# coreperf/rejit

Measured on AMD Instinct MI355X. Metric: GB/s text scanned (regexdna 9 patterns, 50M-line input); matches/s alongside, higher is better.
Workload: dtype u8

## Files before the change

### rejit_amd/csrc/plane_count.hip

```cpp
#include <hip/hip_runtime.h>
#include <hip/hip_ext.h>

#include <cstdlib>

#include "exact_count.h"
#include "kernels.h"
#include "plane_codes.h"
#include "short_walk.h"
#include "stream_load.h"
#include "wave_ops.h"

namespace rejit_amd {

namespace {

constexpr uint64_t kBlock = 2048;
constexpr uint32_t kPieceB = 1024;
constexpr uint32_t kStashWords = (2048 + 16) / 4;
#ifndef RJ_PC_RING
#define RJ_PC_RING 256
#endif
constexpr uint32_t kRing = RJ_PC_RING;

__device__ __forceinline__ uint32_t codes16(const uint4& v, const PlaneCodes& k) {
  const uint32_t s = k.shift;
  return (codes4(v.x, k) >> s) | (codes4(v.y, k) << (8 - s)) | (codes4(v.z, k) << (16 - s)) | (codes4(v.w, k) << (24 - s));
}

struct Raw {
  uint4 a, b;
};

__device__ __forceinline__ void load_block(const uint8_t* block, uint32_t lane_off, Raw& r) {
  r.a = stream_load16(block + lane_off);
  r.b = stream_load16(block + lane_off + kPieceB);
}

__device__ __forceinline__ uint32_t guarded_dword(const uint8_t* text, uint64_t n, uint64_t at) {
  uint32_t v = 0;
#pragma unroll
  for (int k = 0; k < 4; k++)
    if (at + k < n) v |= static_cast<uint32_t>(text[at + k]) << (8 * k);
  return v;
}

template <int NB>
__device__ __forceinline__ uint32_t plane_test(uint32_t ta, uint32_t tb, uint32_t ha, uint32_t hb, const PlaneCountParams& a) {
  constexpr uint32_t kEven = 0x55555555u;
  const uint32_t L = (ta & kEven) | ((tb << 1) & ~kEven);
  const uint32_t H = ((ta >> 1) & kEven) | (tb & ~kEven);
  const uint32_t Ln = (ha & kEven) | ((hb << 1) & ~kEven);
  const uint32_t Hn = ((ha >> 1) & kEven) | (hb & ~kEven);
  register uint32_t q0 asm("v48") = ~(L | H);
  register uint32_t q1 asm("v49") = L & ~H;
  register uint32_t q2 asm("v50") = ~L & H;
  register uint32_t q3 asm("v51") = L & H;
  register uint32_t n0 asm("v52") = ~(Ln | Hn);
  register uint32_t n1 asm("v53") = Ln & ~Hn;
  register uint32_t n2 asm("v54") = ~Ln & Hn;
  register uint32_t n3 asm("v55") = Ln & Hn;
  uint32_t codes = ~a.mask_bits;
  asm volatile("" : "+s"(codes));
  auto code = [&](int b, int i) { return (codes >> (16 * b + 2 * i)) & 3u; };
  uint32_t E[8][NB], Z[NB], O[NB];
#pragma unroll
  for (int half = 0; half < 2; half++) {
    if (NB == 1) {
      if (half == 0) {
      asm volatile(
          "s_set_gpr_idx_on %[c00], 0x3\n"
          "v_mov_b32 %[e00], v48\n"
          "s_set_gpr_idx_idx %[c10]\n"
          "v_alignbit_b32 %[e10], v52, v48, 2\n"
          "s_set_gpr_idx_idx %[c20]\n"
          "v_alignbit_b32 %[e20], v52, v48, 4\n"
          "s_set_gpr_idx_idx %[c30]\n"
          "v_alignbit_b32 %[e30], v52, v48, 6\n"
          "s_set_gpr_idx_off\n"
          : [e00] "=&v"(E[0][0]), [e10] "=&v"(E[1][0]), [e20] "=&v"(E[2][0]), [e30] "=&v"(E[3][0])
          : [c00] "s"(code(0, 0)), [c10] "s"(code(0, 1)), [c20] "s"(code(0, 2)), [c30] "s"(code(0, 3)), "v"(q0), "v"(q1), "v"(q2), "v"(q3), "v"(n0), "v"(n1), "v"(n2), "v"(n3));
      } else {
      asm volatile(
          "s_set_gpr_idx_on %[c40], 0x3\n"
          "v_alignbit_b32 %[e40], v52, v48, 8\n"
          "s_set_gpr_idx_idx %[c50]\n"
          "v_alignbit_b32 %[e50], v52, v48, 10\n"
          "s_set_gpr_idx_idx %[c60]\n"
          "v_alignbit_b32 %[e60], v52, v48, 12\n"
          "s_set_gpr_idx_idx %[c70]\n"
          "v_alignbit_b32 %[e70], v52, v48, 14\n"
          "s_set_gpr_idx_off\n"
          : [e40] "=&v"(E[4][0]), [e50] "=&v"(E[5][0]), [e60] "=&v"(E[6][0]), [e70] "=&v"(E[7][0])
          : [c40] "s"(code(0, 4)), [c50] "s"(code(0, 5)), [c60] "s"(code(0, 6)), [c70] "s"(code(0, 7)), "v"(q0), "v"(q1), "v"(q2), "v"(q3), "v"(n0), "v"(n1), "v"(n2), "v"(n3));
      }
    } else {
      if (half == 0) {
      asm volatile(
          "s_set_gpr_idx_on %[c00], 0x3\n"
          "v_mov_b32 %[e00], v48\n"
          "s_set_gpr_idx_idx %[c01]\n"
          "v_mov_b32 %[e01], v48\n"
          "s_set_gpr_idx_idx %[c10]\n"
          "v_alignbit_b32 %[e10], v52, v48, 2\n"
          "s_set_gpr_idx_idx %[c11]\n"
          "v_alignbit_b32 %[e11], v52, v48, 2\n"
          "s_set_gpr_idx_idx %[c20]\n"
          "v_alignbit_b32 %[e20], v52, v48, 4\n"
          "s_set_gpr_idx_idx %[c21]\n"
          "v_alignbit_b32 %[e21], v52, v48, 4\n"
          "s_set_gpr_idx_idx %[c30]\n"
          "v_alignbit_b32 %[e30], v52, v48, 6\n"
          "s_set_gpr_idx_idx %[c31]\n"
          "v_alignbit_b32 %[e31], v52, v48, 6\n"
          "s_set_gpr_idx_off\n"
          : [e00] "=&v"(E[0][0]), [e01] "=&v"(E[0][1]), [e10] "=&v"(E[1][0]), [e11] "=&v"(E[1][1]), [e20] "=&v"(E[2][0]), [e21] "=&v"(E[2][1]), [e30] "=&v"(E[3][0]), [e31] "=&v"(E[3][1])
          : [c00] "s"(code(0, 0)), [c01] "s"(code(1, 0)), [c10] "s"(code(0, 1)), [c11] "s"(code(1, 1)), [c20] "s"(code(0, 2)), [c21] "s"(code(1, 2)), [c30] "s"(code(0, 3)), [c31] "s"(code(1, 3)), "v"(q0), "v"(q1), "v"(q2), "v"(q3), "v"(n0), "v"(n1), "v"(n2), "v"(n3));
      } else {
      asm volatile(
          "s_set_gpr_idx_on %[c40], 0x3\n"
          "v_alignbit_b32 %[e40], v52, v48, 8\n"
          "s_set_gpr_idx_idx %[c41]\n"
          "v_alignbit_b32 %[e41], v52, v48, 8\n"
          "s_set_gpr_idx_idx %[c50]\n"
          "v_alignbit_b32 %[e50], v52, v48, 10\n"
          "s_set_gpr_idx_idx %[c51]\n"
          "v_alignbit_b32 %[e51], v52, v48, 10\n"
          "s_set_gpr_idx_idx %[c60]\n"
          "v_alignbit_b32 %[e60], v52, v48, 12\n"
          "s_set_gpr_idx_idx %[c61]\n"
          "v_alignbit_b32 %[e61], v52, v48, 12\n"
          "s_set_gpr_idx_idx %[c70]\n"
          "v_alignbit_b32 %[e70], v52, v48, 14\n"
          "s_set_gpr_idx_idx %[c71]\n"
          "v_alignbit_b32 %[e71], v52, v48, 14\n"
          "s_set_gpr_idx_off\n"
          : [e40] "=&v"(E[4][0]), [e41] "=&v"(E[4][1]), [e50] "=&v"(E[5][0]), [e51] "=&v"(E[5][1]), [e60] "=&v"(E[6][0]), [e61] "=&v"(E[6][1]), [e70] "=&v"(E[7][0]), [e71] "=&v"(E[7][1])
          : [c40] "s"(code(0, 4)), [c41] "s"(code(1, 4)), [c50] "s"(code(0, 5)), [c51] "s"(code(1, 5)), [c60] "s"(code(0, 6)), [c61] "s"(code(1, 6)), [c70] "s"(code(0, 7)), [c71] "s"(code(1, 7)), "v"(q0), "v"(q1), "v"(q2), "v"(q3), "v"(n0), "v"(n1), "v"(n2), "v"(n3));
      }
    }
#pragma unroll
    for (int i = 4 * half; i < 4 * half + 4; i++)
#pragma unroll
      for (int b = 0; b < NB; b++) {
        const uint32_t e = E[i][b];
        if (i == 0) {
          Z[b] = e;
        } else if (i == 1) {
          O[b] = Z[b] | e;
          Z[b] &= e;
        } else {
          O[b] = Z[b] | (O[b] & e);
          if (i < 7) Z[b] &= e;
        }
      }
  }
  return NB > 1 ? (O[0] | O[NB - 1]) : O[0];
}


struct Lens {
  uint64_t w[2];
};
static_assert(kMaxFused <= 24, "two words of twelve lengths");
__device__ __forceinline__ uint32_t len_of(const Lens& l, uint32_t p) {
  return static_cast<uint32_t>((p < 12 ? l.w[0] >> (5 * p) : l.w[1] >> (5 * (p - 12))) & 31u);
}

}

template <int NB>
struct ExactShape {
  using Args = PlaneCountParams;
  static constexpr uint32_t kFixedLen = 8;
  static constexpr bool kBlobInLds = false;
  static constexpr bool kList = false;
  static constexpr bool kCapture = true;
  __device__ static __forceinline__ const PlaneCountParams& common(const Args& g) { return g; }
  __device__ static __forceinline__ uint32_t lmax(const Args&) { return 8u; }
  __device__ static __forceinline__ uint32_t offset_of(const Args&, const uint32_t*, uint32_t) { return 0u; }
  __device__ static __forceinline__ uint32_t test(uint32_t ta, uint32_t tb, uint32_t ha, uint32_t hb, const Args& g) { return plane_test<NB>(ta, tb, ha, hb, g); }
  __device__ static __forceinline__ void classify(const Args& a, const uint32_t* table, uint64_t pos, bool have, uint32_t& mask, Lens&) {
    const bool ok = have && pos >= a.sb && pos < a.se && pos + 8 <= a.n;
    uint32_t lo = 0, hi = 0;
    if (ok) {
      __builtin_memcpy(&lo, a.text + pos, 4);
      __builtin_memcpy(&hi, a.text + pos + 4, 4);
    }
    mask = exact_classify<NB>(table, a.base_lo, a.base_hi, lo, hi);
    mask = ok ? mask : 0u;
  }
  __device__ static __forceinline__ void classify_bytes(const Args& a, const uint32_t* table, uint64_t pos, bool have, uint32_t lo, uint32_t hi, uint32_t& mask) {
    const bool ok = have && pos >= a.sb && pos < a.se && pos + 8 <= a.n;
    mask = exact_classify<NB>(table, a.base_lo, a.base_hi, lo, hi);
    mask = ok ? mask : 0u;
  }
};

template <int NB>
struct ListShape {
  using Args = PlaneListParams;
  static constexpr uint32_t kFixedLen = 8;
  static constexpr bool kBlobInLds = false;
  static constexpr bool kList = true;
  static constexpr bool kCapture = false;
  __device__ static __forceinline__ void classify_bytes(const Args&, const uint32_t*, uint64_t, bool, uint32_t, uint32_t, uint32_t& mask) { mask = 0; }
  __device__ static __forceinline__ const PlaneCountParams& common(const Args& g) { return g.c; }
  __device__ static __forceinline__ uint32_t lmax(const Args&) { return 8u; }
  __device__ static __forceinline__ uint32_t offset_of(const Args&, const uint32_t*, uint32_t) { return 0u; }
  __device__ static __forceinline__ uint32_t test(uint32_t ta, uint32_t tb, uint32_t ha, uint32_t hb, const Args& g) { return plane_test<NB>(ta, tb, ha, hb, g.c); }
  __device__ static __forceinline__ void classify(const Args&, const uint32_t*, uint64_t, bool, uint32_t& mask, Lens&) { mask = 0; }
};

namespace {

template <bool TOL>
__device__ __forceinline__ uint32_t general_test(uint32_t ta, uint32_t tb, uint32_t ha, uint32_t hb, const PlaneCountGParams& g) {
  constexpr uint32_t kEven = 0x55555555u;
  const uint32_t L = (ta & kEven) | ((tb << 1) & ~kEven);
  const uint32_t H = ((ta >> 1) & kEven) | (tb & ~kEven);
  const uint32_t Ln = (ha & kEven) | ((hb << 1) & ~kEven);
  const uint32_t Hn = ((ha >> 1) & kEven) | (hb & ~kEven);
  register uint32_t q0 asm("v48") = ~(L | H);
  register uint32_t q1 asm("v49") = L & ~H;
  register uint32_t q2 asm("v50") = ~L & H;
  register uint32_t q3 asm("v51") = L & H;
  register uint32_t q4 asm("v52") = ~0u;
  register uint32_t n0 asm("v56") = ~(Ln | Hn);
  register uint32_t n1 asm("v57") = Ln & ~Hn;
  register uint32_t n2 asm("v58") = ~Ln & Hn;
  register uint32_t n3 asm("v59") = Ln & Hn;
  register uint32_t n4 asm("v60") = ~0u;
  uint32_t c = 0;
#pragma clang loop unroll(disable)
  for (uint32_t b = 0; b < g.c.n_bases; b++) {
    const uint32_t* ix = g.idx[b];
    uint32_t e0, e1, e2, e3, e4, e5, e6, e7;
    asm volatile(
        "s_set_gpr_idx_on %[i0], 0x3\n"
        "v_mov_b32 %[e0], v48\n"
        "s_set_gpr_idx_idx %[i1]\n"
        "v_alignbit_b32 %[e1], v56, v48, 2\n"
        "s_set_gpr_idx_idx %[i2]\n"
        "v_alignbit_b32 %[e2], v56, v48, 4\n"
        "s_set_gpr_idx_idx %[i3]\n"
        "v_alignbit_b32 %[e3], v56, v48, 6\n"
        "s_set_gpr_idx_idx %[i4]\n"
        "v_alignbit_b32 %[e4], v56, v48, 8\n"
        "s_set_gpr_idx_idx %[i5]\n"
        "v_alignbit_b32 %[e5], v56, v48, 10\n"
        "s_set_gpr_idx_idx %[i6]\n"
        "v_alignbit_b32 %[e6], v56, v48, 12\n"
        "s_set_gpr_idx_idx %[i7]\n"
        "v_alignbit_b32 %[e7], v56, v48, 14\n"
        "s_set_gpr_idx_off\n"
        : [e0] "=&v"(e0), [e1] "=&v"(e1), [e2] "=&v"(e2), [e3] "=&v"(e3), [e4] "=&v"(e4), [e5] "=&v"(e5), [e6] "=&v"(e6), [e7] "=&v"(e7)
        : [i0] "s"(ix[0]), [i1] "s"(ix[1]), [i2] "s"(ix[2]), [i3] "s"(ix[3]), [i4] "s"(ix[4]), [i5] "s"(ix[5]), [i6] "s"(ix[6]), [i7] "s"(ix[7]), "v"(q0), "v"(q1), "v"(q2),
          "v"(q3), "v"(q4), "v"(n0), "v"(n1), "v"(n2), "v"(n3), "v"(n4));
    if (TOL) {
      uint32_t Z = e0, O = e0 | e1;
      Z &= e1;
      O = Z | (O & e2);
      Z &= e2;
      O = Z | (O & e3);
      Z &= e3;
      O = Z | (O & e4);
      Z &= e4;
      O = Z | (O & e5);
      Z &= e5;
      O = Z | (O & e6);
      Z &= e6;
      O = Z | (O & e7);
      c |= O;
    } else {
      const uint32_t z0 = e0 & e1 & e2, z1 = e3 & e4 & e5;
      c |= z0 & z1 & e6 & e7;
    }
  }
  return c;
}

}

template <int W, int MAXK, bool TOL>
struct GeneralShape {
  using Args = PlaneCountGParams;
  static constexpr uint32_t kFixedLen = 0;
  static constexpr bool kBlobInLds = true;
  static constexpr bool kList = false;
  static constexpr bool kCapture = false;
  __device__ static __forceinline__ void classify_bytes(const Args&, const uint32_t*, uint64_t, bool, uint32_t, uint32_t, uint32_t& mask) { mask = 0; }
  __device__ static __forceinline__ const PlaneCountParams& common(const Args& g) { return g.c; }
  __device__ static __forceinline__ uint32_t lmax(const Args& g) { return g.lmax; }
  __device__ static __forceinline__ uint32_t offset_of(const Args&, const uint32_t* blob, uint32_t p) {
    return reinterpret_cast<const ClassifyDesc*>(blob)[p].win_offset;
  }
  __device__ static __forceinline__ uint32_t test(uint32_t ta, uint32_t tb, uint32_t ha, uint32_t hb, const Args& g) { return general_test<TOL>(ta, tb, ha, hb, g); }
  __device__ static __forceinline__ void classify(const Args& g, const uint32_t* blob, uint64_t w, bool have, uint32_t& mask, Lens& lens) {
    const PlaneCountParams& a = g.c;
    const ClassifyDesc* desc = reinterpret_cast<const ClassifyDesc*>(blob);
    const uint32_t* tab = blob + g.desc_words;
    uint32_t lo = 0, hi = 0;
    if (have) {
      if (w + 8 <= a.n) {
        __builtin_memcpy(&lo, a.text + w, 4);
        __builtin_memcpy(&hi, a.text + w + 4, 4);
      } else {
        for (uint32_t q = 0; q < 8 && w + q < a.n; q++) {
          const uint32_t c = a.text[w + q];
          if (q < 4) lo |= c << (8 * q);
          else hi |= c << (8 * (q - 4));
        }
      }
    }
    uint32_t todo = 0;
    for (uint32_t p = 0; p < a.n_patterns; p++) {
      const ClassifyDesc& d = desc[p];
      const uint64_t s = w - d.win_offset;
      const bool ok = have && w >= d.win_offset && s >= a.sb && s < a.se && w + d.win_len <= a.n;
      bool win = false;
      for (uint32_t q = 0; q < d.n_windows; q++) win = win || ((((lo ^ d.v0[q]) & d.m0[q]) | ((hi ^ d.v1[q]) & d.m1[q])) == 0);
      todo |= (ok && win) ? 1u << p : 0u;
    }
    mask = 0;
    lens.w[0] = lens.w[1] = 0;
    while (__ballot(todo != 0) != 0) {
      const bool act = todo != 0;
      const uint32_t p = act ? static_cast<uint32_t>(__builtin_ctz(todo)) : 0u;
      todo &= todo - 1;
      const ClassifyDesc& d = desc[p];
      const uint32_t* t0 = tab + d.tab;
      const uint64_t s = w - d.win_offset;
      uint64_t t_lo = 0, t_hi = 0;
      if (act) rj_load16(a.text, a.n, s, &t_lo, &t_hi);
      const uint32_t avail = act ? (a.n - s < 16 ? static_cast<uint32_t>(a.n - s) : 16u) : 0u;
      uint32_t len = 0;
      bool found;
      if (W == 1 || d.n_words <= 1) found = short_longest_lds<1, MAXK>(t0, d, t_lo, t_hi, avail, &len);
      else found = short_longest_lds<W, MAXK>(t0, d, t_lo, t_hi, avail, &len);
      if (found && act && len != 0) {
        mask |= 1u << p;
        if (p < 12) lens.w[0] |= static_cast<uint64_t>(len) << (5 * p);
        else lens.w[1] |= static_cast<uint64_t>(len) << (5 * (p - 12));
      }
    }
  }
};

template <bool TOL>
struct GeneralListShape {
  using Args = PlaneListGParams;
  static constexpr uint32_t kFixedLen = 0;
  static constexpr bool kBlobInLds = false;
  static constexpr bool kList = true;
  static constexpr bool kCapture = false;
  __device__ static __forceinline__ void classify_bytes(const Args&, const uint32_t*, uint64_t, bool, uint32_t, uint32_t, uint32_t& mask) { mask = 0; }
  __device__ static __forceinline__ const PlaneCountParams& common(const Args& g) { return g.g.c; }
  __device__ static __forceinline__ uint32_t lmax(const Args& g) { return g.g.lmax; }
  __device__ static __forceinline__ uint32_t offset_of(const Args&, const uint32_t*, uint32_t) { return 0u; }
  __device__ static __forceinline__ uint32_t test(uint32_t ta, uint32_t tb, uint32_t ha, uint32_t hb, const Args& g) { return general_test<TOL>(ta, tb, ha, hb, g.g); }
  __device__ static __forceinline__ void classify(const Args&, const uint32_t*, uint64_t, bool, uint32_t& mask, Lens&) { mask = 0; }
};

namespace {

struct WaveState {
  uint32_t* ring;
  uint32_t* stash;
  uint32_t head, tail;
  uint32_t acc;
  uint32_t flags;
  uint32_t prev_rel, prev_valid;
  uint32_t* ends;
  uint64_t* list;
  uint32_t list_cap;
  uint64_t list_base;
};
constexpr uint32_t kNoEnd = 0xFFFFFFFFu;

template <bool LIST, bool CAPTURE>
__device__ __forceinline__ void push_block(WaveState& w, uint32_t hm, uint32_t rel_lane, uint32_t block_rel = 0, uint32_t slot = 0) {
  const uint64_t any = __ballot(hm != 0);
  if (any == 0) return;
  auto put = [&](uint32_t idx, uint32_t rel) {
    if (LIST) {
      if (idx < w.list_cap) w.list[idx] = w.list_base + rel;
    } else {
      w.ring[idx & (kRing - 1)] = rel;
      if (CAPTURE) {
        const uint32_t o = rel - block_rel;
        const uint32_t* sw = w.stash + slot * kStashWords + (o >> 2);
        const uint32_t s0 = sw[0], s1 = sw[1], s2 = sw[2];
        w.ring[kRing + (idx & (kRing - 1))] = __builtin_amdgcn_alignbyte(s1, s0, o & 3u);
        w.ring[2 * kRing + (idx & (kRing - 1))] = __builtin_amdgcn_alignbyte(s2, s1, o & 3u);
      }
    }
  };
  const uint32_t hm_a = hm & 0x55555555u, hm_b = hm & 0xAAAAAAAAu;
  const uint64_t several = __ballot((hm & (hm - 1)) != 0);
  if (several == 0) {
    const uint64_t any_a = __ballot(hm_a != 0);
    if (hm != 0) {
      const uint32_t bit = static_cast<uint32_t>(__builtin_ctz(hm));
      const uint32_t at = hm_a != 0 ? lanes_below(any_a) : static_cast<uint32_t>(__popcll(any_a)) + lanes_below(any & ~any_a);
      put(w.tail + at, rel_lane + (bit >> 1) + ((bit & 1u) ? kPieceB : 0u));
    }
    w.tail += static_cast<uint32_t>(__popcll(any));
    return;
  }
  const uint32_t c = __popc(hm_a) | (__popc(hm_b) << 16);
  const uint32_t inc = wave_inclusive_sum(c);
  const uint32_t tots = wave_last_lane(inc);
  const uint32_t tot_a = tots & 0xFFFFu, tot = tot_a + (tots >> 16);
  if (LIST || tot <= kRing) {
    const uint32_t before = inc - c;
    uint32_t idx = w.tail + (before & 0xFFFFu);
    for (uint32_t m = hm_a; m; m &= m - 1, idx++) put(idx, rel_lane + (static_cast<uint32_t>(__builtin_ctz(m)) >> 1));
    idx = w.tail + tot_a + (before >> 16);
    for (uint32_t m = hm_b; m; m &= m - 1, idx++) put(idx, rel_lane + kPieceB + (static_cast<uint32_t>(__builtin_ctz(m)) >> 1));
  }
  w.tail += tot;
}

template <class S>
__device__ __forceinline__ void classify_batch(WaveState& w, uint32_t m, const uint32_t* tab, const typename S::Args& g, uint64_t span_base) {
  const PlaneCountParams& a = S::common(g);
  const int lane = lane_id();
  const bool have = static_cast<uint32_t>(lane) < m;
  const uint32_t rel = w.ring[(w.head + static_cast<uint32_t>(lane)) & (kRing - 1)];
  uint32_t mask;
  Lens lens;
  if constexpr (S::kCapture) {
    const uint32_t lo = w.ring[kRing + ((w.head + static_cast<uint32_t>(lane)) & (kRing - 1))];
    const uint32_t hi = w.ring[2 * kRing + ((w.head + static_cast<uint32_t>(lane)) & (kRing - 1))];
    S::classify_bytes(g, tab, span_base + rel, have, lo, hi, mask);
  } else {
    S::classify(g, tab, span_base + rel, have, mask, lens);
  }
  const uint32_t before = wave_from_lane_below(rel, w.prev_rel);
  const bool has_before = lane > 0 || w.prev_valid != 0;
  const bool close = have && has_before && (rel - before) < S::lmax(g);
  if (__ballot(close && mask != 0) != 0) {
    const uint32_t all_mask = mask;
    const uint32_t suspect = close ? all_mask : 0u;
    for (uint32_t p = 0; p < a.n_patterns; p++) {
      if (__ballot(((suspect >> p) & 1u) != 0) == 0) continue;
      const uint64_t all = __ballot(((all_mask >> p) & 1u) != 0);
      const uint32_t my_len = S::kFixedLen ? S::kFixedLen : len_of(lens, p);
      const uint32_t last_rel = w.ends[4 * p + 2], last_len = w.ends[4 * p + 3];
      uint32_t kept_end = w.ends[4 * p] == kNoEnd ? 0u : static_cast<uint32_t>(__builtin_amdgcn_readfirstlane(static_cast<int>(last_rel + last_len)));
      uint64_t kept = 0;
      for (uint64_t mm = all; mm != 0; mm &= mm - 1) {
        const int i = __builtin_ctzll(mm);
        const uint32_t wi = static_cast<uint32_t>(__builtin_amdgcn_readlane(static_cast<int>(rel), i));
        const uint32_t li = static_cast<uint32_t>(__builtin_amdgcn_readlane(static_cast<int>(my_len), i));
        if (wi >= kept_end) {
          kept |= 1ull << i;
          kept_end = wi + li;
        }
      }
      if ((((all & ~kept) >> lane) & 1ull) != 0) mask &= ~(1u << p);
    }
  }
  for (uint32_t p = 0; p < a.n_patterns; p++) {
    const uint64_t mine = __ballot(((mask >> p) & 1u) != 0);
    if (mine == 0) continue;
    if (lane == static_cast<int>(p)) w.acc += static_cast<uint32_t>(__popcll(mine));
    const int fl = __builtin_ctzll(mine), ll = 63 - __builtin_clzll(mine);
    const uint32_t my_len = S::kFixedLen ? S::kFixedLen : len_of(lens, p);
    const uint32_t first = static_cast<uint32_t>(__builtin_amdgcn_readlane(static_cast<int>(rel), fl));
    const uint32_t last = static_cast<uint32_t>(__builtin_amdgcn_readlane(static_cast<int>(rel), ll));
    const uint32_t first_len = S::kFixedLen ? S::kFixedLen : static_cast<uint32_t>(__builtin_amdgcn_readlane(static_cast<int>(my_len), fl));
    const uint32_t last_len = S::kFixedLen ? S::kFixedLen : static_cast<uint32_t>(__builtin_amdgcn_readlane(static_cast<int>(my_len), ll));
    if (lane == static_cast<int>(p)) {
      if (w.ends[4 * p] == kNoEnd) {
        w.ends[4 * p] = first;
        w.ends[4 * p + 1] = first_len;
      }
      w.ends[4 * p + 2] = last;
      w.ends[4 * p + 3] = last_len;
    }
  }
  w.prev_rel = static_cast<uint32_t>(__builtin_amdgcn_readlane(static_cast<int>(rel), static_cast<int>(m - 1)));
  w.prev_valid = 1;
  w.head += m;
}

template <class S>
__device__ __forceinline__ void check_span_start(WaveState& w, uint32_t m, const uint32_t* tab, const typename S::Args& g, uint64_t span_base) {
  const PlaneCountParams& a = S::common(g);
  const int lane = lane_id();
  const uint32_t reach = S::lmax(g) - 1u;
  const uint32_t rel = w.ring[(w.head + static_cast<uint32_t>(lane)) & (kRing - 1)];
  const bool near = static_cast<uint32_t>(lane) < m && static_cast<uint32_t>(lane) < reach && rel < reach;
  if (__ballot(near) == 0 || span_base == 0) return;
  uint32_t any[2] = {0, 0};
#pragma unroll
  for (int round = 0; round < 2; round++) {
    const uint64_t pos = round == 0 ? span_base + static_cast<uint64_t>(lane) - reach : span_base + rel;
    const bool mine = round == 0 ? (static_cast<uint32_t>(lane) < reach && span_base + static_cast<uint64_t>(lane) >= reach) : near;
    uint32_t mask;
    Lens lens;
    S::classify(g, tab, pos, mine, mask, lens);
    for (uint32_t p = 0; p < a.n_patterns; p++)
      if (__ballot(((mask >> p) & 1u) != 0) != 0) any[round] |= 1u << p;
  }
  if ((any[0] & any[1]) != 0) w.flags |= kPcConflict;
}

template <class S>
__device__ __forceinline__ void blocks_done(WaveState& w, const uint32_t* tab, const typename S::Args& g, uint64_t span_base, bool& first_batch) {
  const PlaneCountParams& a = S::common(g);
  if (w.tail - w.head > kRing) {
    w.flags |= kPcVoid;
    w.head = w.tail;
    return;
  }
  while (w.tail - w.head >= a.batch_at) {
    const uint32_t held = w.tail - w.head;
    const uint32_t m = held < 64u ? held : 64u;
    if (first_batch) check_span_start<S>(w, m, tab, g, span_base);
    first_batch = false;
    classify_batch<S>(w, m, tab, g, span_base);
  }
}

}

template <class S>
__global__ __launch_bounds__(256) void plane_count(typename S::Args g) {
  __shared__ __attribute__((aligned(16))) uint32_t table[kExactTabWords];
  extern __shared__ __attribute__((aligned(16))) uint32_t blob[];
  __shared__ uint32_t rings[4][kRing * (S::kCapture ? 3 : 1)];
  __shared__ __attribute__((aligned(16))) uint32_t stashes[4][S::kCapture ? 2 * kStashWords : 4];
  __shared__ uint32_t ends[4][4 * kExactMaxPatterns];
  __shared__ unsigned long long wave_bounds[4][kExactMaxPatterns][2];
  __shared__ uint32_t wave_counts[4][kExactMaxPatterns];
  __shared__ uint32_t wave_flags[4];
  const PlaneCountParams& a = S::common(g);
  const uint32_t* tab = S::kBlobInLds ? blob : table;
  const int lane = lane_id();
  const uint32_t wid = threadIdx.x >> 6;
  const uint32_t wave = __builtin_amdgcn_readfirstlane(static_cast<uint32_t>((static_cast<uint64_t>(blockIdx.x) * blockDim.x + threadIdx.x) >> 6));
  PlaneCodes k;
  k.shift = a.code_shift;
  k.cmask = 0x03030303u << a.code_shift;
  const uint32_t c0 = static_cast<uint32_t>(a.first_block) + wave * static_cast<uint32_t>(a.span_blocks) + (wave < a.span_extra ? wave : a.span_extra);
  const uint32_t c1 = c0 + static_cast<uint32_t>(a.span_blocks) + (wave < a.span_extra ? 1u : 0u);
  const uint32_t full = static_cast<uint32_t>(a.n / kBlock);
  uint32_t fast_end = full >= 1 ? full - 1 : 0;
  if (fast_end > c1) fast_end = c1;
  if (fast_end < c0) fast_end = c0;
  const uint64_t span_base = static_cast<uint64_t>(c0) * kBlock;
  WaveState w;
  w.ring = rings[wid];
  w.stash = stashes[wid];
  w.ends = ends[wid];
  w.head = w.tail = 0;
  w.acc = 0;
  w.flags = 0;
  w.prev_rel = w.prev_valid = 0;
  w.ends[lane] = kNoEnd;
  w.ends[lane + 64] = kNoEnd;
  w.list = nullptr;
  w.list_cap = 0;
  w.list_base = 0;
  if constexpr (S::kList) {
    if (wave == 0 && lane < kCntSize)
      for (uint32_t p = 0; p < g.n_zero; p++) g.zero_counters[p][lane] = 0;
    w.list = g.hits + static_cast<uint64_t>(wave) * g.region_cap;
    w.list_cap = g.region_cap;
    w.list_base = span_base - g.offset;
  }
  bool first_batch = true;

  const uint32_t last_own = fast_end > c0 ? fast_end - 1 : c0;
  auto blk = [&](uint32_t c) { return a.text + static_cast<uint64_t>(c < last_own ? c : last_own) * kBlock; };
  const uint32_t lane_rel = static_cast<uint32_t>(lane) * 16u;
  Raw ra, rb;
  uint2 behind{0, 0};
  uint32_t c = c0;
  auto stash_put = [&](uint32_t ci, const Raw& r) __attribute__((always_inline)) {
    if constexpr (S::kCapture) {
      uint32_t* sl = w.stash + (ci & 1u) * kStashWords;
      *reinterpret_cast<uint4*>(sl + lane * 4) = r.a;
      *reinterpret_cast<uint4*>(sl + kPieceB / 4 + lane * 4) = r.b;
    }
  };
  auto spill_put = [&](uint32_t ci, uint32_t x, uint32_t y) __attribute__((always_inline)) {
    if constexpr (S::kCapture) {
      if (lane == 0) *reinterpret_cast<uint2*>(w.stash + (ci & 1u) * kStashWords + kBlock / 4) = make_uint2(x, y);
    }
  };
  if (c < fast_end) {
    load_block(blk(c), lane_rel, ra);
    load_block(blk(c + 1), lane_rel, rb);
    behind = *reinterpret_cast<const uint2*>(a.text + static_cast<uint64_t>(fast_end) * kBlock);
  }
  uint64_t clock_in = 0;
  if constexpr (!S::kList) clock_in = __builtin_amdgcn_s_memrealtime();
  if (S::kList) {
  } else if (S::kBlobInLds) {
    const uint4* src = reinterpret_cast<const uint4*>(a.table);
    uint4* dst = reinterpret_cast<uint4*>(blob);
    for (uint32_t i = threadIdx.x; i < a.table_words / 4; i += blockDim.x) dst[i] = src[i];
  } else {
    for (uint32_t i = threadIdx.x; i < kExactTabWords; i += blockDim.x) table[i] = a.table[i];
  }
  __syncthreads();
  if (c < fast_end) {
    uint32_t xa = codes16(ra.a, k), xb = codes16(ra.b, k);
    stash_put(c, ra);
    if (S::kCapture) __builtin_amdgcn_sched_barrier(0);
    load_block(blk(c + 2), lane_rel, ra);
    const uint32_t behind_codes = (codes4(behind.x, k) >> k.shift) | (codes4(behind.y, k) << (8 - k.shift));
    while (c + 1 < fast_end) {
      const uint32_t ya = codes16(rb.a, k), yb = codes16(rb.b, k);
      asm volatile("" ::"v"(ya), "v"(yb));
      stash_put(c + 1, rb);
      spill_put(c, rb.a.x, rb.a.y);
      if (S::kCapture) __builtin_amdgcn_sched_barrier(0);
      if (c + 3 <= last_own) load_block(blk(c + 3), lane_rel, rb);
      {
        const uint32_t ha = wave_from_lane_above(xa, static_cast<uint32_t>(__builtin_amdgcn_readfirstlane(static_cast<int>(xb))));
        const uint32_t hb = wave_from_lane_above(xb, static_cast<uint32_t>(__builtin_amdgcn_readfirstlane(static_cast<int>(ya))));
        const uint32_t hm = S::test(xa, xb, ha, hb, g);
        push_block<S::kList, S::kCapture>(w, hm, (c - c0) * static_cast<uint32_t>(kBlock) + lane_rel, (c - c0) * static_cast<uint32_t>(kBlock), c & 1u);
      }
      __builtin_amdgcn_sched_barrier(0);
      xa = codes16(ra.a, k);
      xb = codes16(ra.b, k);
      asm volatile("" ::"v"(xa), "v"(xb));
      if (c + 2 < fast_end) {
        stash_put(c + 2, ra);
        spill_put(c + 1, ra.a.x, ra.a.y);
      } else {
        spill_put(c + 1, behind.x, behind.y);
      }
      if (S::kCapture) __builtin_amdgcn_sched_barrier(0);
      if (c + 4 <= last_own) load_block(blk(c + 4), lane_rel, ra);
      {
        const uint32_t next0 = c + 2 == fast_end ? behind_codes : static_cast<uint32_t>(__builtin_amdgcn_readfirstlane(static_cast<int>(xa)));
        const uint32_t ha = wave_from_lane_above(ya, static_cast<uint32_t>(__builtin_amdgcn_readfirstlane(static_cast<int>(yb))));
        const uint32_t hb = wave_from_lane_above(yb, next0);
        const uint32_t hm = S::test(ya, yb, ha, hb, g);
        push_block<S::kList, S::kCapture>(w, hm, (c + 1 - c0) * static_cast<uint32_t>(kBlock) + lane_rel, (c + 1 - c0) * static_cast<uint32_t>(kBlock), (c + 1) & 1u);
      }
      __builtin_amdgcn_sched_barrier(0);
      c += 2;
      if (!S::kList && w.tail - w.head >= a.batch_at) blocks_done<S>(w, tab, g, span_base, first_batch);
    }
    if (c + 1 == fast_end) {
      const uint32_t ha = wave_from_lane_above(xa, static_cast<uint32_t>(__builtin_amdgcn_readfirstlane(static_cast<int>(xb))));
      const uint32_t hb = wave_from_lane_above(xb, static_cast<uint32_t>(__builtin_amdgcn_readfirstlane(static_cast<int>(behind_codes))));
      const uint32_t hm = S::test(xa, xb, ha, hb, g);
      spill_put(c, behind.x, behind.y);
      push_block<S::kList, S::kCapture>(w, hm, (c - c0) * static_cast<uint32_t>(kBlock) + lane_rel, (c - c0) * static_cast<uint32_t>(kBlock), c & 1u);
      c++;
    }
    if (!S::kList) blocks_done<S>(w, tab, g, span_base, first_batch);
  }
  for (; c < c1; c++) {
    const uint64_t at = static_cast<uint64_t>(c) * kBlock + lane_rel, bt = at + kPieceB;
    uint4 va, vb;
    va.x = guarded_dword(a.text, a.n, at);
    va.y = guarded_dword(a.text, a.n, at + 4);
    va.z = guarded_dword(a.text, a.n, at + 8);
    va.w = guarded_dword(a.text, a.n, at + 12);
    vb.x = guarded_dword(a.text, a.n, bt);
    vb.y = guarded_dword(a.text, a.n, bt + 4);
    vb.z = guarded_dword(a.text, a.n, bt + 8);
    vb.w = guarded_dword(a.text, a.n, bt + 12);
    const uint32_t g0 = guarded_dword(a.text, a.n, at + 16), g1 = guarded_dword(a.text, a.n, at + 20);
    const uint32_t h0 = guarded_dword(a.text, a.n, bt + 16), h1 = guarded_dword(a.text, a.n, bt + 20);
    const uint32_t ha = (codes4(g0, k) >> k.shift) | (codes4(g1, k) << (8 - k.shift));
    const uint32_t hb = (codes4(h0, k) >> k.shift) | (codes4(h1, k) << (8 - k.shift));
    const uint32_t hm = S::test(codes16(va, k), codes16(vb, k), ha, hb, g);
    if (!S::kList && w.tail - w.head > kRing - 64u) blocks_done<S>(w, tab, g, span_base, first_batch);
    if constexpr (S::kCapture) {
      Raw gr;
      gr.a = va;
      gr.b = vb;
      stash_put(c, gr);
      const uint64_t nb = (static_cast<uint64_t>(c) + 1) * kBlock;
      spill_put(c, guarded_dword(a.text, a.n, nb), guarded_dword(a.text, a.n, nb + 4));
    }
    push_block<S::kList, S::kCapture>(w, hm, (c - c0) * static_cast<uint32_t>(kBlock) + lane_rel, (c - c0) * static_cast<uint32_t>(kBlock), c & 1u);
  }
  if constexpr (S::kList) {
    if (lane == 0) g.hit_counts[wave] = w.tail;
    return;
  }
  if (w.tail - w.head > kRing) {
    w.flags |= kPcVoid;
    w.head = w.tail;
  }
  while (w.tail != w.head) {
    const uint32_t held = w.tail - w.head;
    const uint32_t m = held < 64u ? held : 64u;
    if (first_batch) check_span_start<S>(w, m, tab, g, span_base);
    first_batch = false;
    classify_batch<S>(w, m, tab, g, span_base);
  }
  if (lane < kExactMaxPatterns) {
    const bool real = lane < static_cast<int>(a.n_patterns);
    wave_counts[wid][lane] = real ? w.acc : 0u;
    const uint32_t ef = w.ends[4 * lane], efl = w.ends[4 * lane + 1], el = w.ends[4 * lane + 2], ell = w.ends[4 * lane + 3];
    const uint64_t off = real ? S::offset_of(g, tab, static_cast<uint32_t>(lane)) : 0u;
    wave_bounds[wid][lane][0] = ef != kNoEnd ? ((span_base + ef - off) | (static_cast<unsigned long long>(efl) << kPcLenShift)) : kPcNone;
    wave_bounds[wid][lane][1] = ef != kNoEnd ? ((span_base + el - off) | (static_cast<unsigned long long>(ell) << kPcLenShift)) : kPcNone;
  }
  if (lane == 0) wave_flags[wid] = w.flags;
  __syncthreads();
  if (wid != 0 || lane >= kExactMaxPatterns) return;
  if (lane == 0) *reinterpret_cast<ulonglong2*>(a.wg_clock + static_cast<uint64_t>(blockIdx.x) * 2) = ulonglong2{clock_in, __builtin_amdgcn_s_memrealtime()};
  uint32_t v = wave_counts[0][lane] + wave_counts[1][lane] + wave_counts[2][lane] + wave_counts[3][lane];
  if (lane == kExactMaxPatterns - 1) v = wave_flags[0] | wave_flags[1] | wave_flags[2] | wave_flags[3];
  a.wg_rows[static_cast<uint64_t>(blockIdx.x) * kExactMaxPatterns + lane] = v;
  if (lane < static_cast<int>(a.n_patterns) && v != 0) {
    unsigned long long first = kPcNone, last = kPcNone;
#pragma unroll
    for (int q = 3; q >= 0; q--)
      if (wave_bounds[q][lane][0] != kPcNone) first = wave_bounds[q][lane][0];
#pragma unroll
    for (int q = 0; q < 4; q++)
      if (wave_bounds[q][lane][1] != kPcNone) last = wave_bounds[q][lane][1];
    *reinterpret_cast<ulonglong2*>(a.wg_bounds + (static_cast<uint64_t>(blockIdx.x) * kExactMaxPatterns + lane) * 2) = ulonglong2{first, last};
  }
}

constexpr uint32_t kFinishBatch = 8;
__global__ __launch_bounds__(256, 8) void plane_count_finish(PlaneCountParams a, uint32_t n_wg) {
  __shared__ unsigned long long part[32][kExactMaxPatterns];
  __shared__ uint32_t part_first[32][kExactMaxPatterns], part_last[32][kExactMaxPatterns];
  __shared__ unsigned long long part_clock[4][2];
  __shared__ uint32_t is_last;
  const uint32_t p4 = threadIdx.x & 7u, q = threadIdx.x >> 3;
  const uint32_t lane = threadIdx.x & 63u, wave_id = threadIdx.x >> 6;
  const uint32_t per = (n_wg + gridDim.x - 1) / gridDim.x;
  const uint32_t r_lo = blockIdx.x * per, r_hi = r_lo + per < n_wg ? r_lo + per : n_wg;
  uint32_t sum[4] = {0, 0, 0, 0};
  uint32_t first_row[4] = {0, 0, 0, 0}, last_row[4] = {0, 0, 0, 0};
  const uint4* rows = reinterpret_cast<const uint4*>(a.wg_rows);
  for (uint32_t r = r_lo + q; r < r_hi; r += 32 * kFinishBatch) {
    uint4 v[kFinishBatch];
#pragma unroll
    for (uint32_t i = 0; i < kFinishBatch; i++) {
      const uint32_t rr = r + 32 * i;
      v[i] = rows[static_cast<uint64_t>(rr < r_hi ? rr : r) * 8 + p4];
      if (rr >= r_hi) v[i] = uint4{0, 0, 0, 0};
    }
#pragma unroll
    for (uint32_t i = 0; i < kFinishBatch; i++) {
      const uint32_t rr1 = r + 32 * i + 1;
      const uint32_t c[4] = {v[i].x, v[i].y, v[i].z, v[i].w};
      sum[0] += v[i].x;
      sum[1] += v[i].y;
      sum[2] += v[i].z;
      sum[3] = p4 == 7 ? (sum[3] | v[i].w) : (sum[3] + v[i].w);
#pragma unroll
      for (int k = 0; k < 4; k++) {
        first_row[k] = (c[k] != 0 && first_row[k] == 0) ? rr1 : first_row[k];
        last_row[k] = c[k] != 0 ? rr1 : last_row[k];
      }
    }
  }
#pragma unroll
  for (int i = 0; i < 4; i++) {
    part[q][4 * p4 + i] = sum[i];
    part_first[q][4 * p4 + i] = first_row[i];
    part_last[q][4 * p4 + i] = last_row[i];
  }
  if (lane == 0) {
    part_clock[wave_id][0] = ~0ull;
    part_clock[wave_id][1] = 0;
  }
  const ulonglong2* clocks = reinterpret_cast<const ulonglong2*>(a.wg_clock);
  for (uint32_t r = r_lo + threadIdx.x; r < r_hi; r += 256) {
    const ulonglong2 ck = clocks[r];
    (void)__hip_atomic_fetch_min(&part_clock[wave_id][0], ck.x, __ATOMIC_RELAXED, __HIP_MEMORY_SCOPE_WORKGROUP);
    (void)__hip_atomic_fetch_max(&part_clock[wave_id][1], ck.y, __ATOMIC_RELAXED, __HIP_MEMORY_SCOPE_WORKGROUP);
  }
  __syncthreads();
  if (wave_id == 0) {
    if (lane < kExactMaxPatterns) {
      unsigned long long t = 0;
      uint32_t f = 0, l = 0;
#pragma unroll 4
      for (uint32_t i = 0; i < 32; i++) {
        t = lane == kExactMaxPatterns - 1 ? (t | part[i][lane]) : (t + part[i][lane]);
        const uint32_t pf = part_first[i][lane], pl = part_last[i][lane];
        f = pf != 0 && (f == 0 || pf < f) ? pf : f;
        l = pl > l ? pl : l;
      }
      unsigned long long* g = a.acc + kPcGroupRows + blockIdx.x * kPcGroupWords;
      __hip_atomic_store(&g[lane], t, __ATOMIC_RELAXED, __HIP_MEMORY_SCOPE_AGENT);
      __hip_atomic_store(&g[32 + lane], static_cast<unsigned long long>(f), __ATOMIC_RELAXED, __HIP_MEMORY_SCOPE_AGENT);
      __hip_atomic_store(&g[64 + lane], static_cast<unsigned long long>(l), __ATOMIC_RELAXED, __HIP_MEMORY_SCOPE_AGENT);
    }
    if (lane == 0) {
      unsigned long long in = part_clock[0][0], out = part_clock[0][1];
#pragma unroll
      for (int i = 1; i < 4; i++) {
        in = part_clock[i][0] < in ? part_clock[i][0] : in;
        out = part_clock[i][1] > out ? part_clock[i][1] : out;
      }
      unsigned long long* g = a.acc + kPcGroupRows + blockIdx.x * kPcGroupWords + kPcGroupClock;
      __hip_atomic_store(&g[0], in, __ATOMIC_RELAXED, __HIP_MEMORY_SCOPE_AGENT);
      __hip_atomic_store(&g[1], out, __ATOMIC_RELAXED, __HIP_MEMORY_SCOPE_AGENT);
      const unsigned long long t = __hip_atomic_fetch_add(&a.acc[kPcTicket], 1ull, __ATOMIC_ACQ_REL, __HIP_MEMORY_SCOPE_AGENT);
      is_last = t + 1 == gridDim.x ? 1u : 0u;
      if (t + 1 == gridDim.x) __hip_atomic_store(&a.acc[kPcTicket], 0ull, __ATOMIC_RELAXED, __HIP_MEMORY_SCOPE_AGENT);
    }
  }
  __syncthreads();
  if (!is_last || threadIdx.x >= kExactMaxPatterns) return;
  const uint32_t p = threadIdx.x;
  unsigned long long total = 0;
  uint32_t f = 0, l = 0;
  unsigned long long in = ~0ull, out = 0;
#pragma unroll 2
  for (uint32_t g = 0; g < gridDim.x; g++) {
    const unsigned long long* row = a.acc + kPcGroupRows + g * kPcGroupWords;
    const unsigned long long gi = __hip_atomic_load(&row[kPcGroupClock], __ATOMIC_RELAXED, __HIP_MEMORY_SCOPE_AGENT);
    const unsigned long long go = __hip_atomic_load(&row[kPcGroupClock + 1], __ATOMIC_RELAXED, __HIP_MEMORY_SCOPE_AGENT);
    in = gi < in ? gi : in;
    out = go > out ? go : out;
    const unsigned long long v = __hip_atomic_load(&row[p], __ATOMIC_RELAXED, __HIP_MEMORY_SCOPE_AGENT);
    const uint32_t pf = static_cast<uint32_t>(__hip_atomic_load(&row[32 + p], __ATOMIC_RELAXED, __HIP_MEMORY_SCOPE_AGENT));
    const uint32_t pl = static_cast<uint32_t>(__hip_atomic_load(&row[64 + p], __ATOMIC_RELAXED, __HIP_MEMORY_SCOPE_AGENT));
    total = p == kExactMaxPatterns - 1 ? (total | v) : (total + v);
    f = pf != 0 && (f == 0 || pf < f) ? pf : f;
    l = pl > l ? pl : l;
  }
  if (p == kExactMaxPatterns - 1) {
    a.host_out[kPcHostFlags] = total;
    a.host_out[kPcHostClock] = in;
    a.host_out[kPcHostClock + 1] = out;
  }
  if (p >= a.n_patterns) return;
  unsigned long long first = kPcNone, last = kPcNone;
  if (total != 0 && f != 0) {
    first = a.wg_bounds[(static_cast<uint64_t>(f - 1) * kExactMaxPatterns + p) * 2];
    last = a.wg_bounds[(static_cast<uint64_t>(l - 1) * kExactMaxPatterns + p) * 2 + 1];
  }
  a.host_out[kPcHostCount + p] = total;
  a.host_out[kPcHostBounds + 2 * p] = first;
  a.host_out[kPcHostBounds + 2 * p + 1] = last;
  a.acc[kPcBounds + 2 * p] = first;
  a.acc[kPcBounds + 2 * p + 1] = last;
  a.acc[kPcTotals + p] = total;
}

__global__ void bounds_rows_counts_kernel(BoundsParams a, const unsigned long long* acc, int64_t offset, int first_round, int64_t* rows) {
  const int p = threadIdx.x;
  if (p >= a.n_lists) return;
  uint64_t n = a.count[p];
  int64_t fb = -1, fe = -1, lb = -1, le = -1;
  if (a.spans[p]) {
    const uint64_t* r = a.spans[p];
    if (n) {
      fb = static_cast<int64_t>(r[0]) + offset;
      fe = static_cast<int64_t>(r[1]) + offset;
      lb = static_cast<int64_t>(r[2 * (n - 1)]) + offset;
      le = static_cast<int64_t>(r[2 * (n - 1) + 1]) + offset;
    }
  } else {
    n = acc[kPcTotals + p];
    if (n) {
      const unsigned long long f = acc[kPcBounds + 2 * p], l = acc[kPcBounds + 2 * p + 1];
      const unsigned long long at = (1ull << kPcLenShift) - 1;
      fb = static_cast<int64_t>(f & at) + offset;
      fe = fb + static_cast<int64_t>(f >> kPcLenShift);
      lb = static_cast<int64_t>(l & at) + offset;
      le = lb + static_cast<int64_t>(l >> kPcLenShift);
    }
  }
  rows[8 * p + 0] = static_cast<int64_t>(n);
  if (first_round) {
    rows[8 * p + 1] = fb;
// ... 47 lines not shown
```

Before: 52090.

## Trim register and address overhead in plane-count scan hot loop

Reworks the capture stash so each wave uses two fixed, size-aligned LDS slots with the follower dword placed at slot start, addressed through raw LDS offsets with XOR slot selection. The prefetch pointer now advances incrementally instead of being recomputed per block, lane offsets are combined with OR, and scalar/vector asm hints steer address arithmetic into SGPR base plus VGPR offset. The SGPR pin on pattern codes is limited to the cold tail path, guarded_dword gains a fast unguarded load, and the epilogue reloads output pointers from kernarg to free registers. The goal is lower VALU/SALU address work and register pressure in the main loop. The trade-off is fragile layout assumptions around LDS alignment, the wrapped follower location, and the kernarg offset computation.

```diff
diff --git a/rejit_amd/csrc/plane_count.hip b/rejit_amd/csrc/plane_count.hip
--- a/rejit_amd/csrc/plane_count.hip
+++ b/rejit_amd/csrc/plane_count.hip
@@ -16,7 +16,8 @@
 
 constexpr uint64_t kBlock = 2048;
 constexpr uint32_t kPieceB = 1024;
-constexpr uint32_t kStashWords = (2048 + 16) / 4;
+constexpr uint32_t kStashSlotWords = 2048 / 4;
+constexpr uint32_t kStashBytes = 2 * 2048;
 #ifndef RJ_PC_RING
 #define RJ_PC_RING 256
 #endif
@@ -31,20 +32,28 @@
   uint4 a, b;
 };
 
-__device__ __forceinline__ void load_block(const uint8_t* block, uint32_t lane_off, Raw& r) {
-  r.a = stream_load16(block + lane_off);
-  r.b = stream_load16(block + lane_off + kPieceB);
+__device__ __forceinline__ void load_block(const uint8_t* block, uint32_t lane_off, Raw& r, uint32_t extra = 0) {
+  typedef const __attribute__((address_space(1))) uint8_t* GlobalBytes;
+  GlobalBytes base = (GlobalBytes)block;
+  asm("" : "+s"(base));
+  asm volatile("" : "+v"(lane_off));
+  r.a = stream_load16((const uint8_t*)(base + lane_off + extra));
+  r.b = stream_load16((const uint8_t*)(base + lane_off + extra + kPieceB));
 }
 
 __device__ __forceinline__ uint32_t guarded_dword(const uint8_t* text, uint64_t n, uint64_t at) {
   uint32_t v = 0;
+  if (at + 4 <= n) {
+    __builtin_memcpy(&v, text + at, 4);
+    return v;
+  }
 #pragma unroll
   for (int k = 0; k < 4; k++)
     if (at + k < n) v |= static_cast<uint32_t>(text[at + k]) << (8 * k);
   return v;
 }
 
-template <int NB>
+template <int NB, bool COLD>
 __device__ __forceinline__ uint32_t plane_test(uint32_t ta, uint32_t tb, uint32_t ha, uint32_t hb, const PlaneCountParams& a) {
   constexpr uint32_t kEven = 0x55555555u;
   const uint32_t L = (ta & kEven) | ((tb << 1) & ~kEven);
@@ -60,7 +69,7 @@
   register uint32_t n2 asm("v54") = ~Ln & Hn;
   register uint32_t n3 asm("v55") = Ln & Hn;
   uint32_t codes = ~a.mask_bits;
-  asm volatile("" : "+s"(codes));
+  if (COLD) asm volatile("" : "+s"(codes));
   auto code = [&](int b, int i) { return (codes >> (16 * b + 2 * i)) & 3u; };
   uint32_t E[8][NB], Z[NB], O[NB];
 #pragma unroll
@@ -178,7 +187,8 @@
   __device__ static __forceinline__ const PlaneCountParams& common(const Args& g) { return g; }
   __device__ static __forceinline__ uint32_t lmax(const Args&) { return 8u; }
   __device__ static __forceinline__ uint32_t offset_of(const Args&, const uint32_t*, uint32_t) { return 0u; }
-  __device__ static __forceinline__ uint32_t test(uint32_t ta, uint32_t tb, uint32_t ha, uint32_t hb, const Args& g) { return plane_test<NB>(ta, tb, ha, hb, g); }
+  template <bool COLD = false>
+  __device__ static __forceinline__ uint32_t test(uint32_t ta, uint32_t tb, uint32_t ha, uint32_t hb, const Args& g) { return plane_test<NB, COLD>(ta, tb, ha, hb, g); }
   __device__ static __forceinline__ void classify(const Args& a, const uint32_t* table, uint64_t pos, bool have, uint32_t& mask, Lens&) {
     const bool ok = have && pos >= a.sb && pos < a.se && pos + 8 <= a.n;
     uint32_t lo = 0, hi = 0;
@@ -207,7 +217,8 @@
   __device__ static __forceinline__ const PlaneCountParams& common(const Args& g) { return g.c; }
   __device__ static __forceinline__ uint32_t lmax(const Args&) { return 8u; }
   __device__ static __forceinline__ uint32_t offset_of(const Args&, const uint32_t*, uint32_t) { return 0u; }
-  __device__ static __forceinline__ uint32_t test(uint32_t ta, uint32_t tb, uint32_t ha, uint32_t hb, const Args& g) { return plane_test<NB>(ta, tb, ha, hb, g.c); }
+  template <bool COLD = false>
+  __device__ static __forceinline__ uint32_t test(uint32_t ta, uint32_t tb, uint32_t ha, uint32_t hb, const Args& g) { return plane_test<NB, COLD>(ta, tb, ha, hb, g.c); }
   __device__ static __forceinline__ void classify(const Args&, const uint32_t*, uint64_t, bool, uint32_t& mask, Lens&) { mask = 0; }
 };
 
@@ -294,6 +305,7 @@
   __device__ static __forceinline__ uint32_t offset_of(const Args&, const uint32_t* blob, uint32_t p) {
     return reinterpret_cast<const ClassifyDesc*>(blob)[p].win_offset;
   }
+  template <bool COLD = false>
   __device__ static __forceinline__ uint32_t test(uint32_t ta, uint32_t tb, uint32_t ha, uint32_t hb, const Args& g) { return general_test<TOL>(ta, tb, ha, hb, g); }
   __device__ static __forceinline__ void classify(const Args& g, const uint32_t* blob, uint64_t w, bool have, uint32_t& mask, Lens& lens) {
     const PlaneCountParams& a = g.c;
@@ -357,6 +369,7 @@
   __device__ static __forceinline__ const PlaneCountParams& common(const Args& g) { return g.g.c; }
   __device__ static __forceinline__ uint32_t lmax(const Args& g) { return g.g.lmax; }
   __device__ static __forceinline__ uint32_t offset_of(const Args&, const uint32_t*, uint32_t) { return 0u; }
+  template <bool COLD = false>
   __device__ static __forceinline__ uint32_t test(uint32_t ta, uint32_t tb, uint32_t ha, uint32_t hb, const Args& g) { return general_test<TOL>(ta, tb, ha, hb, g.g); }
   __device__ static __forceinline__ void classify(const Args&, const uint32_t*, uint64_t, bool, uint32_t& mask, Lens&) { mask = 0; }
 };
@@ -366,6 +379,7 @@
 struct WaveState {
   uint32_t* ring;
   uint32_t* stash;
+  uint32_t stash_at;
   uint32_t head, tail;
   uint32_t acc;
   uint32_t flags;
@@ -377,19 +391,32 @@
 };
 constexpr uint32_t kNoEnd = 0xFFFFFFFFu;
 
+__device__ __forceinline__ uint32_t lds_word(uint32_t at) {
+  return *(const __attribute__((address_space(3))) uint32_t*)static_cast<uintptr_t>(at);
+}
+
 template <bool LIST, bool CAPTURE>
-__device__ __forceinline__ void push_block(WaveState& w, uint32_t hm, uint32_t rel_lane, uint32_t block_rel = 0, uint32_t slot = 0) {
+__device__ __forceinline__ void push_block(WaveState& w, uint32_t hm, uint32_t lane_rel, uint32_t block_rel, uint32_t slot = 0) {
   const uint64_t any = __ballot(hm != 0);
   if (any == 0) return;
-  auto put = [&](uint32_t idx, uint32_t rel) {
+  auto put = [&](uint32_t idx, uint32_t o) {
+    const uint32_t rel = block_rel + o;
     if (LIST) {
       if (idx < w.list_cap) w.list[idx] = w.list_base + rel;
     } else {
       w.ring[idx & (kRing - 1)] = rel;
       if (CAPTURE) {
-        const uint32_t o = rel - block_rel;
-        const uint32_t* sw = w.stash + slot * kStashWords + (o >> 2);
-        const uint32_t s0 = sw[0], s1 = sw[1], s2 = sw[2];
+        const uint32_t at = w.stash_at + (o & ~3u);
+        uint32_t s0, s1, s2;
+        if (slot == 0) {
+          s0 = lds_word(at);
+          s1 = lds_word(at + 4);
+          s2 = lds_word(at + 8);
+        } else {
+          s0 = lds_word(at + static_cast<uint32_t>(kBlock));
+          s1 = lds_word((at + 4) ^ static_cast<uint32_t>(kBlock));
+          s2 = lds_word((at + 8) ^ static_cast<uint32_t>(kBlock));
+        }
         w.ring[kRing + (idx & (kRing - 1))] = __builtin_amdgcn_alignbyte(s1, s0, o & 3u);
         w.ring[2 * kRing + (idx & (kRing - 1))] = __builtin_amdgcn_alignbyte(s2, s1, o & 3u);
       }
@@ -402,7 +429,7 @@
     if (hm != 0) {
       const uint32_t bit = static_cast<uint32_t>(__builtin_ctz(hm));
       const uint32_t at = hm_a != 0 ? lanes_below(any_a) : static_cast<uint32_t>(__popcll(any_a)) + lanes_below(any & ~any_a);
-      put(w.tail + at, rel_lane + (bit >> 1) + ((bit & 1u) ? kPieceB : 0u));
+      put(w.tail + at, lane_rel | (bit >> 1) | ((bit & 1u) ? kPieceB : 0u));
     }
     w.tail += static_cast<uint32_t>(__popcll(any));
     return;
@@ -414,9 +441,9 @@
   if (LIST || tot <= kRing) {
     const uint32_t before = inc - c;
     uint32_t idx = w.tail + (before & 0xFFFFu);
-    for (uint32_t m = hm_a; m; m &= m - 1, idx++) put(idx, rel_lane + (static_cast<uint32_t>(__builtin_ctz(m)) >> 1));
+    for (uint32_t m = hm_a; m; m &= m - 1, idx++) put(idx, lane_rel | (static_cast<uint32_t>(__builtin_ctz(m)) >> 1));
     idx = w.tail + tot_a + (before >> 16);
-    for (uint32_t m = hm_b; m; m &= m - 1, idx++) put(idx, rel_lane + kPieceB + (static_cast<uint32_t>(__builtin_ctz(m)) >> 1));
+    for (uint32_t m = hm_b; m; m &= m - 1, idx++) put(idx, lane_rel | kPieceB | (static_cast<uint32_t>(__builtin_ctz(m)) >> 1));
   }
   w.tail += tot;
 }
@@ -531,7 +558,7 @@
   __shared__ __attribute__((aligned(16))) uint32_t table[kExactTabWords];
   extern __shared__ __attribute__((aligned(16))) uint32_t blob[];
   __shared__ uint32_t rings[4][kRing * (S::kCapture ? 3 : 1)];
-  __shared__ __attribute__((aligned(16))) uint32_t stashes[4][S::kCapture ? 2 * kStashWords : 4];
+  __shared__ __attribute__((aligned(S::kCapture ? kStashBytes : 16))) uint32_t stashes[4][S::kCapture ? 2 * kStashSlotWords : 4];
   __shared__ uint32_t ends[4][4 * kExactMaxPatterns];
   __shared__ unsigned long long wave_bounds[4][kExactMaxPatterns][2];
   __shared__ uint32_t wave_counts[4][kExactMaxPatterns];
@@ -554,6 +581,7 @@
   WaveState w;
   w.ring = rings[wid];
   w.stash = stashes[wid];
+  w.stash_at = static_cast<uint32_t>(reinterpret_cast<uintptr_t>((__attribute__((address_space(3))) uint32_t*)stashes[wid]));
   w.ends = ends[wid];
   w.head = w.tail = 0;
   w.acc = 0;
@@ -579,16 +607,16 @@
   Raw ra, rb;
   uint2 behind{0, 0};
   uint32_t c = c0;
-  auto stash_put = [&](uint32_t ci, const Raw& r) __attribute__((always_inline)) {
+  auto stash_put = [&](uint32_t slot, const Raw& r) __attribute__((always_inline)) {
     if constexpr (S::kCapture) {
-      uint32_t* sl = w.stash + (ci & 1u) * kStashWords;
+      uint32_t* sl = w.stash + slot * kStashSlotWords;
       *reinterpret_cast<uint4*>(sl + lane * 4) = r.a;
       *reinterpret_cast<uint4*>(sl + kPieceB / 4 + lane * 4) = r.b;
     }
   };
-  auto spill_put = [&](uint32_t ci, uint32_t x, uint32_t y) __attribute__((always_inline)) {
+  auto follower_put = [&](uint32_t slot, uint32_t x, uint32_t y) __attribute__((always_inline)) {
     if constexpr (S::kCapture) {
-      if (lane == 0) *reinterpret_cast<uint2*>(w.stash + (ci & 1u) * kStashWords + kBlock / 4) = make_uint2(x, y);
+      if (lane == 0) *reinterpret_cast<uint2*>(w.stash + slot * kStashSlotWords) = make_uint2(x, y);
     }
   };
   if (c < fast_end) {
@@ -609,52 +637,49 @@
   __syncthreads();
   if (c < fast_end) {
     uint32_t xa = codes16(ra.a, k), xb = codes16(ra.b, k);
-    stash_put(c, ra);
+    stash_put(0, ra);
     if (S::kCapture) __builtin_amdgcn_sched_barrier(0);
     load_block(blk(c + 2), lane_rel, ra);
     const uint32_t behind_codes = (codes4(behind.x, k) >> k.shift) | (codes4(behind.y, k) << (8 - k.shift));
+    const uint8_t* ahead = a.text + (static_cast<uint64_t>(c) + 3) * kBlock;
     while (c + 1 < fast_end) {
       const uint32_t ya = codes16(rb.a, k), yb = codes16(rb.b, k);
       asm volatile("" ::"v"(ya), "v"(yb));
-      stash_put(c + 1, rb);
-      spill_put(c, rb.a.x, rb.a.y);
+      stash_put(1, rb);
       if (S::kCapture) __builtin_amdgcn_sched_barrier(0);
-      if (c + 3 <= last_own) load_block(blk(c + 3), lane_rel, rb);
+      if (c + 3 <= last_own) load_block(ahead, lane_rel, rb);
       {
         const uint32_t ha = wave_from_lane_above(xa, static_cast<uint32_t>(__builtin_amdgcn_readfirstlane(static_cast<int>(xb))));
         const uint32_t hb = wave_from_lane_above(xb, static_cast<uint32_t>(__builtin_amdgcn_readfirstlane(static_cast<int>(ya))));
         const uint32_t hm = S::test(xa, xb, ha, hb, g);
-        push_block<S::kList, S::kCapture>(w, hm, (c - c0) * static_cast<uint32_t>(kBlock) + lane_rel, (c - c0) * static_cast<uint32_t>(kBlock), c & 1u);
+        push_block<S::kList, S::kCapture>(w, hm, lane_rel, (c - c0) * static_cast<uint32_t>(kBlock), 0u);
       }
       __builtin_amdgcn_sched_barrier(0);
       xa = codes16(ra.a, k);
       xb = codes16(ra.b, k);
       asm volatile("" ::"v"(xa), "v"(xb));
-      if (c + 2 < fast_end) {
-        stash_put(c + 2, ra);
-        spill_put(c + 1, ra.a.x, ra.a.y);
-      } else {
-        spill_put(c + 1, behind.x, behind.y);
-      }
+      if (c + 2 < fast_end) stash_put(0, ra);
+      else follower_put(0, behind.x, behind.y);
       if (S::kCapture) __builtin_amdgcn_sched_barrier(0);
-      if (c + 4 <= last_own) load_block(blk(c + 4), lane_rel, ra);
+      if (c + 4 <= last_own) load_block(ahead, lane_rel, ra, static_cast<uint32_t>(kBlock));
       {
         const uint32_t next0 = c + 2 == fast_end ? behind_codes : static_cast<uint32_t>(__builtin_amdgcn_readfirstlane(static_cast<int>(xa)));
         const uint32_t ha = wave_from_lane_above(ya, static_cast<uint32_t>(__builtin_amdgcn_readfirstlane(static_cast<int>(yb))));
         const uint32_t hb = wave_from_lane_above(yb, next0);
         const uint32_t hm = S::test(ya, yb, ha, hb, g);
-        push_block<S::kList, S::kCapture>(w, hm, (c + 1 - c0) * static_cast<uint32_t>(kBlock) + lane_rel, (c + 1 - c0) * static_cast<uint32_t>(kBlock), (c + 1) & 1u);
+        push_block<S::kList, S::kCapture>(w, hm, lane_rel, (c + 1 - c0) * static_cast<uint32_t>(kBlock), 1u);
       }
       __builtin_amdgcn_sched_barrier(0);
       c += 2;
+      ahead += 2 * kBlock;
       if (!S::kList && w.tail - w.head >= a.batch_at) blocks_done<S>(w, tab, g, span_base, first_batch);
     }
     if (c + 1 == fast_end) {
       const uint32_t ha = wave_from_lane_above(xa, static_cast<uint32_t>(__builtin_amdgcn_readfirstlane(static_cast<int>(xb))));
       const uint32_t hb = wave_from_lane_above(xb, static_cast<uint32_t>(__builtin_amdgcn_readfirstlane(static_cast<int>(behind_codes))));
       const uint32_t hm = S::test(xa, xb, ha, hb, g);
-      spill_put(c, behind.x, behind.y);
-      push_block<S::kList, S::kCapture>(w, hm, (c - c0) * static_cast<uint32_t>(kBlock) + lane_rel, (c - c0) * static_cast<uint32_t>(kBlock), c & 1u);
+      follower_put(1, behind.x, behind.y);
+      push_block<S::kList, S::kCapture>(w, hm, lane_rel, (c - c0) * static_cast<uint32_t>(kBlock), 0u);
       c++;
     }
     if (!S::kList) blocks_done<S>(w, tab, g, span_base, first_batch);
@@ -674,17 +699,17 @@
     const uint32_t h0 = guarded_dword(a.text, a.n, bt + 16), h1 = guarded_dword(a.text, a.n, bt + 20);
     const uint32_t ha = (codes4(g0, k) >> k.shift) | (codes4(g1, k) << (8 - k.shift));
     const uint32_t hb = (codes4(h0, k) >> k.shift) | (codes4(h1, k) << (8 - k.shift));
-    const uint32_t hm = S::test(codes16(va, k), codes16(vb, k), ha, hb, g);
+    const uint32_t hm = S::template test<true>(codes16(va, k), codes16(vb, k), ha, hb, g);
     if (!S::kList && w.tail - w.head > kRing - 64u) blocks_done<S>(w, tab, g, span_base, first_batch);
     if constexpr (S::kCapture) {
       Raw gr;
       gr.a = va;
       gr.b = vb;
-      stash_put(c, gr);
+      stash_put((c - c0) & 1u, gr);
       const uint64_t nb = (static_cast<uint64_t>(c) + 1) * kBlock;
-      spill_put(c, guarded_dword(a.text, a.n, nb), guarded_dword(a.text, a.n, nb + 4));
-    }
-    push_block<S::kList, S::kCapture>(w, hm, (c - c0) * static_cast<uint32_t>(kBlock) + lane_rel, (c - c0) * static_cast<uint32_t>(kBlock), c & 1u);
+      follower_put((c - c0 + 1) & 1u, guarded_dword(a.text, a.n, nb), guarded_dword(a.text, a.n, nb + 4));
+    }
+    push_block<S::kList, S::kCapture>(w, hm, lane_rel, (c - c0) * static_cast<uint32_t>(kBlock), (c - c0) & 1u);
   }
   if constexpr (S::kList) {
     if (lane == 0) g.hit_counts[wave] = w.tail;
@@ -712,10 +737,17 @@
   if (lane == 0) wave_flags[wid] = w.flags;
   __syncthreads();
   if (wid != 0 || lane >= kExactMaxPatterns) return;
-  if (lane == 0) *reinterpret_cast<ulonglong2*>(a.wg_clock + static_cast<uint64_t>(blockIdx.x) * 2) = ulonglong2{clock_in, __builtin_amdgcn_s_memrealtime()};
+  const __attribute__((address_space(4))) char* again = (const __attribute__((address_space(4))) char*)__builtin_amdgcn_kernarg_segment_ptr();
+  asm volatile("" : "+s"(again));
+  again += reinterpret_cast<const char*>(&a) - reinterpret_cast<const char*>(&g);
+  const auto* rows = reinterpret_cast<const __attribute__((address_space(4))) PlaneCountParams*>(again);
+  uint32_t* const wg_rows = rows->wg_rows;
+  unsigned long long* const wg_bounds = rows->wg_bounds;
+  unsigned long long* const wg_clock = rows->wg_clock;
+  if (lane == 0) *reinterpret_cast<ulonglong2*>(wg_clock + static_cast<uint64_t>(blockIdx.x) * 2) = ulonglong2{clock_in, __builtin_amdgcn_s_memrealtime()};
   uint32_t v = wave_counts[0][lane] + wave_counts[1][lane] + wave_counts[2][lane] + wave_counts[3][lane];
   if (lane == kExactMaxPatterns - 1) v = wave_flags[0] | wave_flags[1] | wave_flags[2] | wave_flags[3];
-  a.wg_rows[static_cast<uint64_t>(blockIdx.x) * kExactMaxPatterns + lane] = v;
+  wg_rows[static_cast<uint64_t>(blockIdx.x) * kExactMaxPatterns + lane] = v;
   if (lane < static_cast<int>(a.n_patterns) && v != 0) {
     unsigned long long first = kPcNone, last = kPcNone;
 #pragma unroll
@@ -724,7 +756,7 @@
 #pragma unroll
     for (int q = 0; q < 4; q++)
       if (wave_bounds[q][lane][1] != kPcNone) last = wave_bounds[q][lane][1];
-    *reinterpret_cast<ulonglong2*>(a.wg_bounds + (static_cast<uint64_t>(blockIdx.x) * kExactMaxPatterns + lane) * 2) = ulonglong2{first, last};
+    *reinterpret_cast<ulonglong2*>(wg_bounds + (static_cast<uint64_t>(blockIdx.x) * kExactMaxPatterns + lane) * 2) = ulonglong2{first, last};
   }
 }
 
```

Result: faster. 53640, median of 6 (+3.0%).
